# probcomp/PClean

Measured on AMD Instinct MI355X. Metric: rows/sec per Gibbs sweep on 1M-row synthetic hospital; F1 vs ground truth, higher is better.
Workload: dtype f64

## Files before the change

### pclean_amd/csrc/commit.hip

```cpp
#include <hip/hip_runtime.h>

#include <algorithm>
#include <cmath>

#define PCC_DEVICE
__device__ long long pcc_prof_t[64];
__device__ int pcc_prof_n;
#define PCC_STAMP(name)                                                   \
  do {                                                                    \
    if (tid == 0 && blockIdx.x == 0 && pcc_prof_n < 64) pcc_prof_t[pcc_prof_n++] = (long long)wall_clock64(); \
  } while (0)
#define PCC_CUR_SEPARATE
#include "commit_core.h"
#include "sweep_state.h"

struct PccRefresh {
  const int64_t* counts;
  double* logc_full;
  double* logc_m1;
  const double* lut;
  int32_t lut_n, stride;
};
struct PccRefreshAll {
  PccRefresh t[PCC_MAX_SLOTS];
};
struct PccSums {
  unsigned long long total[PCC_MAX_SLOTS], live[PCC_MAX_SLOTS], maxc[PCC_MAX_SLOTS];
  int32_t lut_overflow, pad;
};

struct CommitSlot {
  int table_id = -1;
  int stride = 0;
  bool state_set = false;
  DevBuf<uint8_t> live;
  DevBuf<int32_t> free_stack, gflag, gscan, glist, origin, chg;
  DevBuf<double> lut;
  int lut_n = 0;
  double lut_discount = 0.0;
  bool lut_valid = false;
  int64_t max_count = 0;
};

struct CommitState {
  bool enabled = false;
  int n_slots = 0, n_blocks = 0, n_plans = 0;
  int slot_of_table[PCLEAN_MAX_TABLES];
  int plan_block[PCC_MAX_BLOCKS];
  CommitSlot slot[PCC_MAX_SLOTS];
  PccTable h_tables[PCC_MAX_SLOTS];
  PccPlan h_plans[PCC_MAX_BLOCKS];
  DevBuf<PccTable> d_tables;
  DevBuf<PccPlan> d_plans;
  DevBuf<PccBlock> d_blocks;
  DevBuf<int32_t> d_colmap[PCC_MAX_BLOCKS];
  DevBuf<int32_t> d_states;
  bool tables_dirty = true, plans_dirty = true;
  int kcap[PCC_MAX_BLOCKS];
  DevBuf<int32_t> ht[PCC_MAX_BLOCKS], rep[PCC_MAX_BLOCKS], flags[PCC_MAX_BLOCKS], scan[PCC_MAX_BLOCKS], base[PCC_MAX_BLOCKS],
      newid[PCC_MAX_BLOCKS], recpos[PCC_MAX_BLOCKS];
  DevBuf<PccResult> d_res;
  DevBuf<PccSums> d_sums;
  DevBuf<int> d_bar;
  int bar_count = 0;
  int cap_m[PCC_MAX_BLOCKS] = {0}, cap_k[PCC_MAX_BLOCKS] = {0};
  DevBuf<int32_t> seg, seg_all, g_counts2;
  DevBuf<int32_t> g_moved[PCC_MAX_BLOCKS], g_choice[PCC_MAX_BLOCKS], g_new[PCC_MAX_BLOCKS], g_chosen[PCC_MAX_BLOCKS],
      g_vals[PCC_MAX_BLOCKS];
  DevBuf<PccBlock> d_blocks_g;
  PccBlock* h_blocks_g = nullptr;
  int32_t* h_g_counts2 = nullptr;
  PccBlock* h_blocks = nullptr;
  PccResult* h_res = nullptr;
  PccSums* h_sums = nullptr;
  int32_t* h_states = nullptr;
};

static CommitState* cst(pclean_ctx* ctx) {
  if (!ctx->commit_state) ctx->commit_state = new CommitState();
  return (CommitState*)ctx->commit_state;
}

void pclean_commit_state_free(pclean_ctx* ctx) {
  if (!ctx->commit_state) return;
  CommitState* c = (CommitState*)ctx->commit_state;
  for (auto& s : c->slot) {
    s.live.release(); s.free_stack.release(); s.gflag.release(); s.gscan.release(); s.glist.release(); s.origin.release(); s.chg.release();
    s.lut.release();
  }
  c->d_tables.release(); c->d_plans.release(); c->d_blocks.release(); c->d_states.release(); c->d_res.release();
  c->d_sums.release();
  c->d_bar.release();
  for (int b = 0; b < PCC_MAX_BLOCKS; ++b) {
    c->d_colmap[b].release(); c->ht[b].release(); c->rep[b].release(); c->flags[b].release(); c->scan[b].release();
    c->base[b].release(); c->newid[b].release(); c->recpos[b].release();
  }
  if (c->h_blocks) (void)hipHostFree(c->h_blocks);
  if (c->h_res) (void)hipHostFree(c->h_res);
  if (c->h_sums) (void)hipHostFree(c->h_sums);
  if (c->h_states) (void)hipHostFree(c->h_states);
  if (c->h_blocks_g) (void)hipHostFree(c->h_blocks_g);
  if (c->h_g_counts2) (void)hipHostFree(c->h_g_counts2);
  c->seg.release(); c->seg_all.release(); c->g_counts2.release(); c->d_blocks_g.release();
  for (int b = 0; b < PCC_MAX_BLOCKS; ++b) {
    c->g_moved[b].release(); c->g_choice[b].release(); c->g_new[b].release(); c->g_chosen[b].release(); c->g_vals[b].release();
  }
  ctx->dev_cur.release();
  delete c;
  ctx->commit_state = nullptr;
}

void pclean_commit_table_reuploaded(pclean_ctx* ctx, int table_id) {
  if (!ctx->commit_state || table_id < 0 || table_id >= PCLEAN_MAX_TABLES) return;
  CommitState* c = (CommitState*)ctx->commit_state;
  if (!c->enabled) return;
  const int si = c->slot_of_table[table_id];
  if (si >= 0) c->slot[si].state_set = false;
}

__global__ __launch_bounds__(1024) void pcc_commit_kernel(PccTable* tb, int n_slots, const PccPlan* plans, const PccBlock* blocks,
                                                          int n_blocks, PccResult* res, int gathered) {
  __shared__ int32_t part[1025];
  if (threadIdx.x == 0) pcc_prof_n = 0;
  if (threadIdx.x == 0 && !gathered) res->fallback_in = 0;
  if (threadIdx.x == 0)
    for (int s = 0; s < n_slots; ++s) {
      tb[s].state[PCC_ST_COLS_CHANGED] = 0;
      tb[s].state[PCC_ST_CREATED] = 0;
      tb[s].state[PCC_ST_DELETED] = 0;
      tb[s].state[PCC_ST_NCHG] = 0;
    }
  pcc_commit(tb, n_slots, plans, blocks, n_blocks, res, part, (int)threadIdx.x, (int)blockDim.x);
}

__device__ void pcc_mw_barrier(int* ctr, int target) {
  __syncthreads();
  if (threadIdx.x == 0) {
    __threadfence();
    atomicAdd(ctr, 1);
    while (__hip_atomic_load(ctr, __ATOMIC_RELAXED, __HIP_MEMORY_SCOPE_AGENT) < target) __builtin_amdgcn_s_sleep(1);
    __threadfence();
  }
  __syncthreads();
}
__global__ __launch_bounds__(1024) void pcc_commit_mw_kernel(PccTable* tb, int n_slots, const PccPlan* plans, const PccBlock* blocks,
                                                             int n_blocks, PccResult* res, int gathered, int* bar, int bar0) {
  __shared__ int32_t part[1025];
  const int tid = (int)threadIdx.x, nt = (int)blockDim.x, bi = (int)blockIdx.x;
  if (bi == 0 && tid == 0) {
    pcc_prof_n = 0;
    if (!gathered) res->fallback_in = 0;
    for (int s = 0; s < n_slots; ++s) {
      tb[s].state[PCC_ST_COLS_CHANGED] = 0;
      tb[s].state[PCC_ST_CREATED] = 0;
      tb[s].state[PCC_ST_DELETED] = 0;
      tb[s].state[PCC_ST_NCHG] = 0;
    }
    res->fallback = res->fallback_in;
    res->n_changed = 0;
    for (int s = 0; s < PCC_MAX_SLOTS; ++s) res->alloc_upper[s] = 0;
    for (int b = 0; b < PCC_MAX_BLOCKS; ++b) res->n_records[b] = res->n_distinct[b] = res->n_nested[b] = 0;
  }
  pcc_mw_barrier(bar, bar0 + n_blocks);
  if (res->fallback) {
    if (tid == 0) atomicAdd(bar, 1);
    return;
  }
  pcc_prepare_block(tb, plans[bi], blocks[bi], bi, res, tid, nt);
  __syncthreads();
  if (tid == 0) {
    const PccPlan& pl = plans[bi];
    for (int u = 0; u < pl.n_used; ++u) {
      const int s = pl.used_slot[u];
      const int a = res->alloc_upper[s];
      if (a == 0) continue;
      if (tb[s].state[PCC_ST_NHW] + (a > tb[s].state[PCC_ST_NFREE] ? a - tb[s].state[PCC_ST_NFREE] : 0) > tb[s].stride)
        atomicOr(&res->fallback, PCC_FB_CAPACITY);
    }
  }
  pcc_mw_barrier(bar, bar0 + 2 * n_blocks);
  if (res->fallback) return;
  pcc_apply_block(tb, plans[bi], blocks[bi], bi, res, part, tid, nt);
}

__global__ __launch_bounds__(256) void pcc_cur_kernel(const PccBlock* blocks, const PccResult* res) {
  if (res->fallback) return;
  pcc_update_cur(blocks[blockIdx.y], (int)(blockIdx.x * 256 + threadIdx.x), (int)(gridDim.x * 256));
}

struct PccGathered {
  int32_t* g_moved[PCC_MAX_BLOCKS];
  int32_t* g_choice[PCC_MAX_BLOCKS];
  int32_t* g_new[PCC_MAX_BLOCKS];
  int32_t* g_chosen[PCC_MAX_BLOCKS];
  int32_t* g_vals[PCC_MAX_BLOCKS];
  int32_t cap_out_m[PCC_MAX_BLOCKS], cap_out_k[PCC_MAX_BLOCKS];
};
__global__ __launch_bounds__(256) void pcc_pack_kernel(PccSegLayout L, const PccBlock* blocks, int empty, int32_t* seg) {
  pcc_pack(L, (int)blockIdx.y, blocks[blockIdx.y], empty, seg, (int)(blockIdx.x * 256 + threadIdx.x), (int)(gridDim.x * 256));
}
__global__ __launch_bounds__(256) void pcc_merge_kernel(PccSegLayout L, int n_ranks, const int32_t* all, PccGathered g,
                                                        int32_t* counts2, PccResult* res) {
  const int p = blockIdx.y;
  pcc_merge(L, p, n_ranks, all, g.cap_out_m[p], g.cap_out_k[p], g.g_moved[p], g.g_choice[p], g.g_new[p], g.g_chosen[p], g.g_vals[p],
            counts2 + 2 * p, &res->fallback_in, (int)(blockIdx.x * 256 + threadIdx.x), (int)(gridDim.x * 256),
            blockIdx.x == 0 ? counts2 + 2 * PCC_MAX_BLOCKS + 2 * p : nullptr);
}

__global__ void pcc_live_kernel(int n, const int64_t* counts, uint8_t* live) {
  const int r = blockIdx.x * blockDim.x + threadIdx.x;
  if (r < n) live[r] = counts[r] > 0 ? 1 : 0;
}

// ... 80 lines not shown
  for (int s = 0; s < sc->n_slots; ++s) {
    c->slot[s].table_id = sc->slot_table[s];
    c->h_tables[s] = sc->tables[s];
  }
  for (int p = 0; p < sc->n_plans; ++p) {
    c->plan_block[p] = sc->plan_block[p];
    c->h_plans[p] = sc->plans[p];
    const Block& b = ctx->block[sc->plan_block[p]];
    if (c->d_colmap[p].alloc(std::max<size_t>(b.colmap.size(), 2))) {
      delete sc;
      return pclean_fail(ctx, PCLEAN_ERR_HIP, "device alloc failed");
    }
    if (!b.colmap.empty()) {
      const hipError_t e = hipMemcpy(c->d_colmap[p].p, b.colmap.data(), b.colmap.size() * 4, hipMemcpyHostToDevice);
      if (e != hipSuccess) {
        delete sc;
        return pclean_fail(ctx, PCLEAN_ERR_HIP, "hipMemcpy failed: %s", hipGetErrorString(e));
      }
    }
    c->h_plans[p].colmap = c->d_colmap[p].p;
    c->kcap[p] = 0;
  }
  delete sc;
  if (c->d_tables.alloc(PCC_MAX_SLOTS) || c->d_plans.alloc(PCC_MAX_BLOCKS) || c->d_blocks.alloc(PCC_MAX_BLOCKS) ||
      c->d_states.alloc(PCC_MAX_SLOTS * PCC_ST_WORDS) || c->d_res.alloc(1) || c->d_sums.alloc(1))
    return pclean_fail(ctx, PCLEAN_ERR_HIP, "device alloc failed");
  if (!c->h_blocks) {
    HIPCHK(ctx, hipHostMalloc((void**)&c->h_blocks, sizeof(PccBlock) * PCC_MAX_BLOCKS, hipHostMallocDefault));
    HIPCHK(ctx, hipHostMalloc((void**)&c->h_res, sizeof(PccResult), hipHostMallocDefault));
    HIPCHK(ctx, hipHostMalloc((void**)&c->h_sums, sizeof(PccSums), hipHostMallocDefault));
    HIPCHK(ctx, hipHostMalloc((void**)&c->h_states, sizeof(int32_t) * PCC_MAX_SLOTS * PCC_ST_WORDS, hipHostMallocDefault));
  }
  c->tables_dirty = c->plans_dirty = true;
  c->enabled = true;
  *supported = 1;
  return PCLEAN_OK;
}

extern "C" int pclean_commit_n_slots(pclean_ctx* ctx, int32_t* n_slots, int32_t* table_ids) {
  if (!ctx || !n_slots) return PCLEAN_ERR_ARG;
  CommitState* c = cst(ctx);
  *n_slots = c->enabled ? c->n_slots : 0;
  if (table_ids)
    for (int s = 0; s < *n_slots; ++s) table_ids[s] = c->slot[s].table_id;
  return PCLEAN_OK;
}

extern "C" int pclean_commit_set_table_state(pclean_ctx* ctx, int32_t table_id, int32_t n_hw, int32_t n_free,
                                             const int32_t* free_stack) {
  if (!ctx || table_id < 0 || table_id >= PCLEAN_MAX_TABLES || n_hw < 0 || n_free < 0 || (n_free > 0 && !free_stack))
    return pclean_fail(ctx, PCLEAN_ERR_ARG, "pclean_commit_set_table_state: bad arguments");
  CommitState* c = cst(ctx);
  if (!c->enabled || c->slot_of_table[table_id] < 0)
    return pclean_fail(ctx, PCLEAN_ERR_STATE, "pclean_commit_set_table_state: table %d is not part of an enabled commit", table_id);
  HIPCHK(ctx, hipSetDevice(ctx->device));
  const int si = c->slot_of_table[table_id];
  CommitSlot& s = c->slot[si];
  CandTable& t = ctx->cand[table_id];
  if (!t.valid || n_hw > t.n_rows || n_free > n_hw)
    return pclean_fail(ctx, PCLEAN_ERR_ARG, "pclean_commit_set_table_state: table %d: %d rows in use, capacity %d", table_id, n_hw,
                       t.n_rows);
  const size_t st = std::max(t.n_rows, 1);
  if (s.live.alloc(st) || s.free_stack.alloc(st) || s.gflag.alloc(st) || s.gscan.alloc(st) || s.glist.alloc(st) ||
      s.origin.alloc(4 * st) || s.chg.alloc(st))
    return pclean_fail(ctx, PCLEAN_ERR_HIP, "device alloc failed");
  s.stride = t.n_rows;
// ... 68 lines not shown
  HIPCHK(ctx, hipMemcpyAsync(state8, c->d_states.p + (size_t)si * PCC_ST_WORDS, PCC_ST_WORDS * 4, hipMemcpyDeviceToHost, ctx->stream));
  if (cols && st) HIPCHK(ctx, hipMemcpyAsync(cols, t.cols.p, st * t.n_cols * 4, hipMemcpyDeviceToHost, ctx->stream));
  if (counts && st) HIPCHK(ctx, hipMemcpyAsync(counts, t.counts.p, st * 8, hipMemcpyDeviceToHost, ctx->stream));
  if (live && st) HIPCHK(ctx, hipMemcpyAsync(live, s.live.p, st, hipMemcpyDeviceToHost, ctx->stream));
  if (free_stack && st) HIPCHK(ctx, hipMemcpyAsync(free_stack, s.free_stack.p, st * 4, hipMemcpyDeviceToHost, ctx->stream));
  if (origin && st) {
    HIPCHK(ctx, hipMemcpyAsync(origin, s.origin.p, st * 16, hipMemcpyDeviceToHost, ctx->stream));
    HIPCHK(ctx, hipMemsetAsync(s.origin.p, 0, st * 16, ctx->stream));
  }
  HIPCHK(ctx, hipStreamSynchronize(ctx->stream));
  if (cols && st && t.h_cols_stale && t.h_cols.size() == st * (size_t)t.n_cols) {
    memcpy(t.h_cols.data(), cols, st * (size_t)t.n_cols * 4);
    t.h_cols_stale = false;
  }
  return PCLEAN_OK;
}

static int ensure_lut(pclean_ctx* ctx, CommitSlot& s, int64_t need) {
  const CandTable& t = ctx->cand[s.table_id];
  if (s.lut_valid && s.lut_discount == t.discount && s.lut_n > need) return PCLEAN_OK;
  const int64_t n = std::max<int64_t>(4096, 2 * need + 1024);
  if (n > (int64_t)1 << 30) return pclean_fail(ctx, PCLEAN_ERR_CAPACITY, "reference count beyond the log table");
  if (s.lut.alloc((size_t)n)) return pclean_fail(ctx, PCLEAN_ERR_HIP, "device alloc failed");
  std::vector<double> h((size_t)n);
  h[0] = -INFINITY;
  for (int64_t cc = 1; cc < n; ++cc) h[(size_t)cc] = std::log((double)cc - t.discount);
  HIPCHK(ctx, hipMemcpy(s.lut.p, h.data(), (size_t)n * sizeof(double), hipMemcpyHostToDevice));
  s.lut_n = (int)n;
  s.lut_discount = t.discount;
  s.lut_valid = true;
  return PCLEAN_OK;
}

static int launch_refresh(pclean_ctx* ctx, CommitState* c) {
  PccRefreshAll ra{};
  int max_stride = 1;
  for (int si = 0; si < c->n_slots; ++si) {
    CommitSlot& s = c->slot[si];
    CandTable& t = ctx->cand[s.table_id];
    ra.t[si] = PccRefresh{t.counts.p, t.logc_full.p, t.logc_m1.p, s.lut.p, s.lut_n, t.n_rows};
    max_stride = std::max(max_stride, t.n_rows);
  }
  { const int rcz = dev_zero(ctx, c->d_sums.p, sizeof(PccSums)); if (rcz) return rcz; }
  hipLaunchKernelGGL(pcc_refresh_kernel, dim3((max_stride + 255) / 256, c->n_slots), dim3(256), 0, ctx->stream, ra, c->d_res.p,
                     c->d_sums.p);
  {
    const int rcs = d2h_small(ctx, c->h_sums, c->d_sums.p, sizeof(PccSums));
    if (rcs) return rcs;
  }
  return PCLEAN_OK;
}

static int commit_device_impl(pclean_ctx* ctx, int32_t n_blocks, uint32_t sweep_idx, bool dist, bool local_empty,
                              int32_t max_local_rows, pclean_commit_summary* out);
extern "C" int pclean_commit_device(pclean_ctx* ctx, int32_t n_blocks, uint32_t sweep_idx, pclean_commit_summary* out) {
  if (ctx && ctx->comm_ranks > 1)
    return pclean_fail(ctx, PCLEAN_ERR_STATE, "pclean_commit_device: several ranks commit through pclean_commit_device_dist "
                                              "(every rank's moved rows and new-row records are gathered on the device first)");
  return commit_device_impl(ctx, n_blocks, sweep_idx, false, false, 0, out);
}
extern "C" int pclean_commit_device_dist(pclean_ctx* ctx, int32_t n_blocks, uint32_t sweep_idx, int32_t local_empty,
                                         int32_t max_local_rows, pclean_commit_summary* out) {
  if (!ctx || !ctx->rccl_comm || ctx->comm_ranks < 1 || max_local_rows < 0)
    return pclean_fail(ctx, PCLEAN_ERR_STATE, "pclean_commit_device_dist: pclean_comm_init first");
  return commit_device_impl(ctx, n_blocks, sweep_idx, true, local_empty != 0, max_local_rows, out);
}
static int commit_device_impl(pclean_ctx* ctx, int32_t n_blocks, uint32_t sweep_idx, bool dist, bool local_empty,
                              int32_t max_local_rows, pclean_commit_summary* out) {
  if (!ctx || !out) return pclean_fail(ctx, PCLEAN_ERR_ARG, "pclean_commit_device: bad arguments");
  CommitState* c = cst(ctx);
  SweepState* s = st(ctx);
  if (!c->enabled || c->n_blocks != n_blocks) return pclean_fail(ctx, PCLEAN_ERR_STATE, "pclean_commit_device: pclean_commit_enable first");
  if (!local_empty && (!s->outputs_pending || !s->last_dev_cur || s->last_blocks != n_blocks))
    return pclean_fail(ctx, PCLEAN_ERR_STATE, "pclean_commit_device: needs a pclean_sweep with device-resident referents "
                                              "(cur == NULL) and deferred outputs right before it");
  if (dist && (!ctx->dev_cur_valid || ctx->dev_cur_blocks != n_blocks))
// ... 14 lines not shown
        const int32_t* ov = ctx->cand[b.nodes[i].table].cols.p;
        if (pl.opt_vals[i] != ov) {
          pl.opt_vals[i] = ov;
          c->plans_dirty = true;
        }
      }
  }
  for (int si = 0; si < c->n_slots; ++si) {
    CandTable& t = ctx->cand[c->slot[si].table_id];
    PccTable& pt = c->h_tables[si];
    if (pt.cols != t.cols.p || pt.counts != t.counts.p) {
      pt.cols = t.cols.p;
      pt.counts = t.counts.p;
      c->tables_dirty = true;
    }
    int rc = ensure_lut(ctx, c->slot[si], c->slot[si].max_count + 1);
    if (rc) return rc;
  }
  if (c->tables_dirty) {
    HIPCHK(ctx, hipMemcpyAsync(c->d_tables.p, c->h_tables, sizeof(PccTable) * PCC_MAX_SLOTS, hipMemcpyHostToDevice, ctx->stream));
    HIPCHK(ctx, hipStreamSynchronize(ctx->stream));
    c->tables_dirty = false;
  }
  if (c->plans_dirty) {
    HIPCHK(ctx, hipMemcpyAsync(c->d_plans.p, c->h_plans, sizeof(PccPlan) * PCC_MAX_BLOCKS, hipMemcpyHostToDevice, ctx->stream));
    HIPCHK(ctx, hipStreamSynchronize(ctx->stream));
    c->plans_dirty = false;
  }
  for (int p = 0; p < c->n_plans; ++p) {
    const int bi = c->plan_block[p];
    const Block& b = ctx->block[bi];
    BlockRun& r = s->run[bi];
    const PccPlan& pl = c->h_plans[p];
    if (c->kcap[p] < 16384) c->kcap[p] = 16384;
    const int kcap = c->kcap[p];
    int hsz = 1;
    while (hsz < 4 * kcap) hsz <<= 1;
    if (c->ht[p].alloc(hsz) || c->rep[p].alloc(kcap) || c->flags[p].alloc(kcap) || c->scan[p].alloc(kcap) ||
        c->base[p].alloc((size_t)kcap * pl.n_used) || c->newid[p].alloc(kcap) || c->recpos[p].alloc(kcap))
      return pclean_fail(ctx, PCLEAN_ERR_HIP, "device alloc failed");
    PccBlock& pb = c->h_blocks[p];
    pb.N = N;
    pb.nn = (int)b.nodes.size();
    pb.block_id = bi;
    pb.sweep_idx = (int32_t)sweep_idx;
    pb.row_lo = (int32_t)(s->row_offset + ctx->active_begin);
    pb.pad0 = 0;
    pb.choice = r.choice.p;
    pb.chosen = s->chosen.p;
    pb.chosen_newpos = r.chosen_newpos.p;
    pb.vals = r.vals.p;
    pb.moved_list = r.moved_list.p;
    pb.new_list = r.new_list.p;
    pb.counts2 = s->tail_counts.p + 2 * bi;
    pb.cur = local_empty ? nullptr : const_cast<int32_t*>(s->last_cur_base) + (size_t)bi * s->last_cur_ld;
    pb.moved_choice = nullptr;
    pb.rec_chosen = nullptr;
    pb.delta = ctx->cand[b.nodes[0].table].stats.p;
    pb.kcap = kcap;
    pb.hmask = hsz - 1;
    pb.ht = c->ht[p].p;
    pb.rep = c->rep[p].p;
    pb.flags = c->flags[p].p;
    pb.scan = c->scan[p].p;
    pb.base = c->base[p].p;
    pb.newid = c->newid[p].p;
    pb.recpos = c->recpos[p].p;
  }
  HIPCHK(ctx, hipMemcpyAsync(c->d_blocks.p, c->h_blocks, sizeof(PccBlock) * c->n_plans, hipMemcpyHostToDevice, ctx->stream));
  const PccBlock* commit_blocks = c->d_blocks.p;
  bool stats_reduced = false;
  int cur_rows = N;
  if (dist) {
    PccSegLayout L{};
    L.n_plans = c->n_plans;
    int32_t off = 0;
    for (int p = 0; p < c->n_plans; ++p) {
      if (c->cap_m[p] <= 0) c->cap_m[p] = std::max(max_local_rows, 16);
      if (c->cap_k[p] <= 0) c->cap_k[p] = std::max(max_local_rows, 16);
      L.off[p] = off;
      L.cap_m[p] = c->cap_m[p];
      L.cap_k[p] = c->cap_k[p];
      L.nn[p] = (int)ctx->block[c->plan_block[p]].nodes.size();
      off += pcc_seg_words(L.cap_m[p], L.cap_k[p], L.nn[p]);
    }
    L.seg_words = off;
    if (c->seg.alloc((size_t)off) || c->seg_all.alloc((size_t)off * world) || c->g_counts2.alloc(4 * PCC_MAX_BLOCKS) ||
        c->d_blocks_g.alloc(PCC_MAX_BLOCKS))
      return pclean_fail(ctx, PCLEAN_ERR_HIP, "device alloc failed");
    if (!c->h_blocks_g) {
      HIPCHK(ctx, hipHostMalloc((void**)&c->h_blocks_g, sizeof(PccBlock) * PCC_MAX_BLOCKS, hipHostMallocDefault));
      HIPCHK(ctx, hipHostMalloc((void**)&c->h_g_counts2, sizeof(int32_t) * 4 * PCC_MAX_BLOCKS, hipHostMallocDefault));
    }
    PccGathered G{};
    for (int p = 0; p < c->n_plans; ++p) {
      const size_t om = (size_t)L.cap_m[p] * world, ok = (size_t)L.cap_k[p] * world;
      if (c->g_moved[p].alloc(om) || c->g_choice[p].alloc(om) || c->g_new[p].alloc(ok) || c->g_chosen[p].alloc(ok) ||
          c->g_vals[p].alloc(ok * L.nn[p]))
        return pclean_fail(ctx, PCLEAN_ERR_HIP, "device alloc failed");
      G.g_moved[p] = c->g_moved[p].p;
      G.g_choice[p] = c->g_choice[p].p;
      G.g_new[p] = c->g_new[p].p;
// ... 34 lines not shown
      pb.chosen_newpos = nullptr;
      pb.vals = c->g_vals[p].p;
      pb.moved_list = c->g_moved[p].p;
      pb.new_list = c->g_new[p].p;
      pb.moved_choice = c->g_choice[p].p;
      pb.rec_chosen = c->g_chosen[p].p;
      pb.counts2 = c->g_counts2.p + 2 * p;
      pb.cur = ctx->dev_cur.p + (size_t)bi * ctx->n_rows;
    }
    HIPCHK(ctx, hipMemcpyAsync(c->d_blocks_g.p, c->h_blocks_g, sizeof(PccBlock) * c->n_plans, hipMemcpyHostToDevice, ctx->stream));
    { const int rcz = dev_zero(ctx, c->d_res.p, sizeof(PccResult)); if (rcz) return rcz; }
    int32_t tids[PCC_MAX_BLOCKS];
    int n_t = 0;
    for (int p = 0; p < c->n_plans; ++p) {
      const int t = ctx->block[c->plan_block[p]].nodes[0].table;
      bool seen = false;
      for (int k = 0; k < n_t; ++k) seen |= tids[k] == t;
      if (!seen) tids[n_t++] = t;
    }
    int rc = pclean_comm_allreduce_stats_queue(ctx, n_t, tids, local_empty ? 1 : 0);
    if (rc) return rc;
    stats_reduced = true;
    hipLaunchKernelGGL(pcc_pack_kernel, dim3(64, c->n_plans), dim3(256), 0, ctx->stream, L, c->d_blocks.p, local_empty ? 1 : 0,
                       c->seg.p);
    rc = pclean_comm_allgather_i32(ctx, c->seg.p, c->seg_all.p, (size_t)L.seg_words);
    if (rc) return rc;
    hipLaunchKernelGGL(pcc_merge_kernel, dim3(64, c->n_plans), dim3(256), 0, ctx->stream, L, world, c->seg_all.p, G, c->g_counts2.p,
                       c->d_res.p);
    HIPCHK(ctx, hipMemcpyAsync(c->h_g_counts2, c->g_counts2.p, sizeof(int32_t) * 4 * PCC_MAX_BLOCKS, hipMemcpyDeviceToHost, ctx->stream));
    commit_blocks = c->d_blocks_g.p;
    cur_rows = 0;
    for (int p = 0; p < c->n_plans; ++p) cur_rows = std::max<int64_t>(cur_rows, (int64_t)L.cap_m[p] * world);
  }
  static const bool no_mw = getenv("PCLEAN_COMMIT_ONE_WG") != nullptr;
  bool all_exclusive = c->n_plans > 1 && !no_mw;
  for (int p = 0; p < c->n_plans; ++p) all_exclusive = all_exclusive && c->h_plans[p].exclusive != 0;
  if (all_exclusive && !c->d_bar.p) {
    if (c->d_bar.alloc(16)) return pclean_fail(ctx, PCLEAN_ERR_HIP, "device alloc failed");
    HIPCHK(ctx, hipMemsetAsync(c->d_bar.p, 0, 16 * sizeof(int), ctx->stream));
    c->bar_count = 0;
  }
  if (all_exclusive) {
    if (c->bar_count > (1 << 30)) {
      HIPCHK(ctx, hipMemsetAsync(c->d_bar.p, 0, 16 * sizeof(int), ctx->stream));
      c->bar_count = 0;
    }
    hipLaunchKernelGGL(pcc_commit_mw_kernel, dim3(c->n_plans), dim3(1024), 0, ctx->stream, c->d_tables.p, c->n_slots, c->d_plans.p,
                       commit_blocks, c->n_plans, c->d_res.p, dist ? 1 : 0, c->d_bar.p, c->bar_count);
    c->bar_count += 2 * c->n_plans;
  } else {
    hipLaunchKernelGGL(pcc_commit_kernel, dim3(1), dim3(1024), 0, ctx->stream, c->d_tables.p, c->n_slots, c->d_plans.p,
                       commit_blocks, c->n_plans, c->d_res.p, dist ? 1 : 0);
  }
  hipLaunchKernelGGL(pcc_cur_kernel, dim3(std::max(1, std::min(1024, (cur_rows + 255) / 256)), c->n_plans), dim3(256), 0, ctx->stream,
                     commit_blocks, c->d_res.p);
  int rc = launch_refresh(ctx, c);
  if (rc) return rc;
  rc = d2h_small(ctx, c->h_res, c->d_res.p, sizeof(PccResult));
  if (!rc) rc = d2h_small(ctx, c->h_states, c->d_states.p, sizeof(int32_t) * PCC_MAX_SLOTS * PCC_ST_WORDS);
  if (rc) return rc;
  rc = pclean_sweep_finish_queue(ctx);
  if (!rc) rc = d2h_flush(ctx);
  if (rc) return rc;
  HIPCHK(ctx, hipGetLastError());
  HIPCHK(ctx, hipStreamSynchronize(ctx->stream));
  rc = pclean_sweep_finish_synced(ctx);
  if (rc) return rc;
  static const bool prof = getenv("PCLEAN_COMMIT_PROF") != nullptr;
  if (prof) {
    long long t[64];
    int n = 0;
    (void)hipMemcpyFromSymbol(&n, HIP_SYMBOL(pcc_prof_n), sizeof n);
    (void)hipMemcpyFromSymbol(t, HIP_SYMBOL(pcc_prof_t), sizeof t);
    fprintf(stderr, "[pclean] commit kernel phases (us since start; 100 MHz clock):");
    for (int i = 1; i < n && i < 64; ++i) fprintf(stderr, " %.1f", (double)(t[i] - t[0]) / 100.0);
    fprintf(stderr, "  (records %d %d, moved %d %d)\n", c->h_res->n_records[0], c->h_res->n_records[1], s->h_counts[0], s->h_counts[2]);
  }
  out->fallback = c->h_res->fallback;
  out->n_changed = c->h_res->n_changed;
  out->n_slots = c->n_slots;
  out->stats_reduced = stats_reduced ? 1 : 0;
  for (int p = 0; p < c->n_plans; ++p) {
    out->n_records[c->plan_block[p]] = c->h_res->n_records[p];
    out->n_distinct[c->plan_block[p]] = c->h_res->n_distinct[p];
    if (2 * c->h_res->n_records[p] > c->kcap[p]) c->kcap[p] = 2 * c->h_res->n_records[p];
    if (dist) {
      c->cap_m[p] = out->fallback ? 0 : std::max(1024, 4 * c->h_g_counts2[2 * PCC_MAX_BLOCKS + 2 * p] + 256);
      c->cap_k[p] = out->fallback ? 0 : std::max(256, 4 * c->h_g_counts2[2 * PCC_MAX_BLOCKS + 2 * p + 1] + 256);
    }
  }
  if (dist && !out->fallback) {
    int64_t moved = 0;
    for (int p = 0; p < c->n_plans; ++p) moved += c->h_g_counts2[2 * p];
    out->n_changed = (int32_t)moved;
  }
  if (out->fallback) return PCLEAN_OK;
  for (int guard = 0; c->h_sums->lut_overflow && guard < 4; ++guard) {
    for (int si = 0; si < c->n_slots; ++si) {
      rc = ensure_lut(ctx, c->slot[si], (int64_t)c->h_sums->maxc[si] + 1);
      if (rc) return rc;
    }
// ... 47 lines not shown
```

### pclean_amd/csrc/commit_core.h

```cpp
#pragma once
#include <stdint.h>

#ifdef PCC_DEVICE
#define PCC_FN __device__
#define PCC_BARRIER() __syncthreads()
#define PCC_ADD64(p, v) atomicAdd((unsigned long long*)(p), (unsigned long long)(long long)(v))
#define PCC_ADD32(p, v) atomicAdd((int*)(p), (int)(v))
#define PCC_FETCH_ADD32(p, v) atomicAdd((int*)(p), (int)(v))
#define PCC_OR32(p, v) atomicOr((int*)(p), (int)(v))
#define PCC_MIN32(p, v) atomicMin((int*)(p), (int)(v))
#define PCC_CAS32(p, cmp, v) atomicCAS((int*)(p), (int)(cmp), (int)(v))
#else
#define PCC_FN static inline
#define PCC_BARRIER() ((void)0)
#define PCC_ADD64(p, v) (*(p) += (int64_t)(v))
#define PCC_ADD32(p, v) (*(p) += (int32_t)(v))
static inline int32_t pcc_fetch_add32_host(int32_t* p, int32_t v) {
  const int32_t old = *p;
  *p += v;
  return old;
}
#define PCC_FETCH_ADD32(p, v) pcc_fetch_add32_host((p), (v))
#define PCC_OR32(p, v) (*(p) |= (int32_t)(v))
#define PCC_MIN32(p, v) (*(p) = (*(p) < (int32_t)(v) ? *(p) : (int32_t)(v)))
// ... 270 lines not shown
      fr_slot[depth] = t.fk_slot[q];
      fr_n[depth] = L2;
      fr_next[depth] = 0;
      ++depth;
    }
  }
}

PCC_FN void pcc_mark_reuse(const PccTable* tb, const PccPlan& pl, const PccBlock& b, int k, bool pending_delta, int tid, int nt) {
  const PccTable& root = tb[pl.used_slot[0]];
  for (int j = tid; j < k; j += nt) {
    int32_t fl = b.flags[j];
    int32_t fresh = 0;
    if ((fl & PCC_F_FIRST) && (fl & PCC_F_SIMPLE)) {
      const int32_t* v = pcc_record(b, j);
      int32_t row[PCC_MAX_NODES];
      (void)pcc_new_nodes(pl, v, row);
      const int old = b.cur[b.new_list[j]];
      bool same = old >= 0 && root.live[old] && root.counts[old] + (pending_delta ? b.delta[old] : 0) == 0;
      for (int c = 0; c < root.n_cols && same; ++c)
        same = root.cols[(size_t)c * root.stride + old] == pcc_col_value(tb, pl, v, row, 0, c);
      if (same) {
        b.newid[j] = old;
        b.flags[j] = fl | PCC_F_REUSE;
      } else {
        fresh = 1;
      }
    }
    b.scan[j] = fresh;
  }
  PCC_BARRIER();
}

PCC_FN void pcc_prepare_block(const PccTable* tb, const PccPlan& pl, const PccBlock& b, int bi, PccResult* res, int tid, int nt) {
  const int k = b.counts2[1];
  if (tid == 0) {
    res->n_records[bi] = k;
    res->n_distinct[bi] = 0;
    res->n_nested[bi] = 0;
  }
  if (k > b.kcap) {
    if (tid == 0) PCC_OR32(&res->fallback, PCC_FB_RECORDS);
    return;
  }
  if (k == 0) return;
  for (int j = tid; j < k; j += nt) b.recpos[j] = b.chosen_newpos ? b.chosen_newpos[b.new_list[j]] : j;
  int hm = b.hmask < 63 ? b.hmask : 63;
  while (hm + 1 < 4 * k && hm < b.hmask) hm = 2 * hm + 1;
  const uint32_t hmask = (uint32_t)hm;
  for (int i = tid; i <= hm; i += nt) b.ht[i] = -1;
  PCC_BARRIER();
  for (int j = tid; j < k; j += nt) {
    const int32_t* v = pcc_record(b, j);
    uint32_t s = pcc_hash(b, v) & hmask;
    for (;;) {
      int32_t c = b.ht[s];
      if (c < 0) {
        c = PCC_CAS32(&b.ht[s], -1, j);
        if (c < 0) break;
      }
      if (pcc_same(b, pcc_record(b, c), v)) {
        PCC_MIN32(&b.ht[s], j);
        break;
      }
      s = (s + 1) & hmask;
    }
  }
  PCC_BARRIER();
  for (int j = tid; j < k; j += nt) {
    const int32_t* v = pcc_record(b, j);
    uint32_t s = pcc_hash(b, v) & hmask;
    for (;;) {
      const int32_t c = b.ht[s];
      if (pcc_same(b, pcc_record(b, c), v)) {
        b.rep[j] = c;
        break;
      }
      s = (s + 1) & hmask;
    }
    int32_t fl = 0;
    if (b.rep[j] == j) {
      fl = PCC_F_FIRST | PCC_F_SIMPLE;
      int32_t row[PCC_MAX_NODES];
      const uint64_t mask = pcc_new_nodes(pl, v, row);
      if (mask != 1ull) {
        fl &= ~PCC_F_SIMPLE;
        PCC_ADD32(&res->n_nested[bi], 1);
      }
      for (int p = 0; p < pl.n_fk_nodes; ++p) {
        const int f = pl.fk_post[p];
        if (((mask >> f) & 1ull) && !(f == 0 && pl.exclusive)) PCC_ADD32(&res->alloc_upper[pl.slot[f]], 1);
      }
      for (int l = 0; l < pl.n_nodes; ++l)
        if (pl.kind[l] == 1 && pl.dummy_val[l] != 0 && ((mask >> pl.parent[l]) & 1ull) && v[l] >= 0 &&
            pl.opt_vals[l][v[l]] == pl.dummy_val[l] - 1)
          PCC_OR32(&res->fallback, PCC_FB_DUMMY);
      PCC_ADD32(&res->n_distinct[bi], 1);
    }
    b.flags[j] = fl;
  }
  PCC_BARRIER();
  if (pl.exclusive) {
    pcc_mark_reuse(tb, pl, b, k, true, tid, nt);
    for (int j = tid; j < k; j += nt)
      if ((b.flags[j] & PCC_F_FIRST) && !(b.flags[j] & PCC_F_REUSE)) PCC_ADD32(&res->alloc_upper[pl.used_slot[0]], 1);
    PCC_BARRIER();
  }
}

PCC_FN void pcc_update_cur(const PccBlock& b, int tid, int nt) {
  const int k = b.counts2[1], n_moved = b.counts2[0];
  for (int m = tid; m < n_moved; m += nt) {
    const int r = b.moved_list[m];
    const int c = b.moved_choice ? b.moved_choice[m] : b.choice[r];
    if (c >= 0) b.cur[r] = c;
  }
  for (int j = tid; j < k; j += nt) b.cur[b.new_list[j]] = b.newid[j];
}

PCC_FN void pcc_apply_block(PccTable* tb, const PccPlan& pl, const PccBlock& b, int bi, PccResult* res, int32_t* part, int tid,
                            int nt) {
  const int k = b.counts2[1], n_moved = b.counts2[0];
  const int U = pl.n_used;
  PccTable& root = tb[pl.used_slot[0]];
  {
    const int n0 = root.state[PCC_ST_NHW];
    for (int r = tid; r < n0; r += nt) root.counts[r] += b.delta[r];
    PCC_BARRIER();
  }
  PCC_STAMP("delta");
  if (k > 0) {
  if (!pl.exclusive) pcc_mark_reuse(tb, pl, b, k, false, tid, nt);
  const int32_t n_simple = pcc_excl_scan(b.scan, k, part, tid, nt);
  for (int j = tid; j < k; j += nt) b.base[(size_t)j * U] = b.scan[j];
  PCC_BARRIER();
  PCC_STAMP("reuse+scan");
  int32_t total[PCC_MAX_SLOTS];
  for (int u = 0; u < U; ++u) total[u] = u == 0 ? n_simple : 0;
  if (res->n_nested[bi] > 0)
  for (int u = 0; u < U; ++u) {
// ... 150 lines not shown
      for (int r = 0; r < n_ranks; ++r) {
        const int32_t* o = all + (size_t)r * L.seg_words + L.off[p];
        mm = o[0] > mm ? o[0] : mm;
        mk = o[1] > mk ? o[1] : mk;
      }
      rank_max[0] = mm;
      rank_max[1] = mk;
    }
  }
  if (bad) return;
  int base_m = 0, base_k = 0;
  for (int r = 0; r < n_ranks; ++r) {
    const int32_t* o = all + (size_t)r * L.seg_words + L.off[p];
    const int32_t* mrow = o + 4;
    const int32_t* mch = mrow + cm;
    const int32_t* nrow = mch + cm;
    const int32_t* nchs = nrow + ck;
    const int32_t* rec = nchs + ck;
    const int nm = o[0], nk = o[1];
    for (int m = tid; m < nm; m += nt) {
      g_moved[base_m + m] = mrow[m];
      g_choice[base_m + m] = mch[m];
    }
    for (int j = tid; j < nk; j += nt) {
      g_new[base_k + j] = nrow[j];
      g_chosen[base_k + j] = nchs[j];
    }
    for (int x = tid; x < nk * nn; x += nt) g_vals[(size_t)base_k * nn + x] = rec[x];
    base_m += nm;
    base_k += nk;
  }
}

PCC_FN void pcc_commit(PccTable* tb, int n_slots, const PccPlan* plans, const PccBlock* blocks, int n_blocks, PccResult* res,
                       int32_t* part, int tid, int nt) {
  if (tid == 0) {
    res->fallback = res->fallback_in;
    res->n_changed = 0;
    for (int s = 0; s < PCC_MAX_SLOTS; ++s) res->alloc_upper[s] = 0;
    for (int bi = 0; bi < PCC_MAX_BLOCKS; ++bi) res->n_records[bi] = res->n_distinct[bi] = res->n_nested[bi] = 0;
  }
  PCC_BARRIER();
  PCC_STAMP("start");
  if (res->fallback) return;
  for (int bi = 0; bi < n_blocks; ++bi) {
    pcc_prepare_block(tb, plans[bi], blocks[bi], bi, res, tid, nt);
    PCC_STAMP("prepare");
  }
  PCC_BARRIER();
  if (tid == 0)
    for (int s = 0; s < n_slots; ++s) {
      const int a = res->alloc_upper[s];
      if (a == 0) continue;
      const int from_free = tb[s].n_blocks_using <= 1 ? tb[s].state[PCC_ST_NFREE] : 0;
      if (tb[s].state[PCC_ST_NHW] + (a > from_free ? a - from_free : 0) > tb[s].stride) res->fallback |= PCC_FB_CAPACITY;
    }
  PCC_BARRIER();
  if (res->fallback) return;
  for (int bi = 0; bi < n_blocks; ++bi) pcc_apply_block(tb, plans[bi], blocks[bi], bi, res, part, tid, nt);
}

#ifndef PCC_DEVICE_ONLY
struct PccNodeIn {
  int32_t kind, table, child_begin, n_children, parent, parent_fk_col, colmap_begin, dummy_value;
};
static inline void pcc_post_order(const PccNodeIn* nodes, const int32_t* children, int f, PccPlan& pl) {
  for (int c = 0; c < nodes[f].n_children; ++c) {
    const int g = children[nodes[f].child_begin + c];
    if (nodes[g].kind == 0) pcc_post_order(nodes, children, g, pl);
  }
  pl.fk_post[pl.n_fk_nodes++] = f;
}
static inline int pcc_build_plan(const PccNodeIn* nodes, int n_nodes, const int32_t* children, const int32_t* slot_of_table,
                                 PccPlan& pl) {
  if (n_nodes > PCC_MAX_NODES || n_nodes < 1 || nodes[0].kind != 0) return -1;
  pl.n_nodes = n_nodes;
  pl.n_fk_nodes = 0;
  pl.n_used = 0;
  pl.track = 0;
  for (int i = 0; i < n_nodes; ++i) {
    pl.kind[i] = nodes[i].kind;
    pl.parent[i] = nodes[i].parent;
    pl.parent_fk_col[i] = nodes[i].parent_fk_col;
    pl.cmb[i] = nodes[i].colmap_begin;
    pl.dummy_val[i] = nodes[i].kind == 1 ? nodes[i].dummy_value : 0;
    pl.slot[i] = -1;
    pl.node_used[i] = -1;
    pl.opt_vals[i] = nullptr;
    if (nodes[i].kind == 1 && nodes[i].dummy_value != 0) pl.track = 1;
    if (nodes[i].kind == 0) {
      const int s = slot_of_table[nodes[i].table];
      if (s < 0) return -2;
// ... 137 lines not shown
```

Before: 408.2 million.

## Split commit prepare phase into grid-wide kernels and skip redundant block uploads

The per-block prepare step (hash-table init, insert, classify, reuse marking) used to run inside the single-workgroup or one-WG-per-block commit kernel. It now runs as three grid-wide kernels launched across many workgroups, and the commit kernel only does the apply phase. The prep-init kernel also zeroes the sums buffer, replacing a separate memset, and the host skips re-uploading the PccBlock descriptors when they are unchanged. The cost is two extra kernel launches and a host-side memcmp. The old narrow path is kept behind an environment variable.

```diff
diff --git a/pclean_amd/csrc/commit.hip b/pclean_amd/csrc/commit.hip
--- a/pclean_amd/csrc/commit.hip
+++ b/pclean_amd/csrc/commit.hip
@@ -6,9 +6,10 @@
 #define PCC_DEVICE
 __device__ long long pcc_prof_t[64];
 __device__ int pcc_prof_n;
+__device__ int pcc_prof_wg;
 #define PCC_STAMP(name)                                                   \
   do {                                                                    \
-    if (tid == 0 && blockIdx.x == 0 && pcc_prof_n < 64) pcc_prof_t[pcc_prof_n++] = (long long)wall_clock64(); \
+    if (tid == 0 && (int)blockIdx.x == pcc_prof_wg && pcc_prof_n < 64) pcc_prof_t[pcc_prof_n++] = (long long)wall_clock64(); \
   } while (0)
 #define PCC_CUR_SEPARATE
 #include "commit_core.h"
@@ -63,6 +64,8 @@
   DevBuf<PccSums> d_sums;
   DevBuf<int> d_bar;
   int bar_count = 0;
+  PccBlock up_blocks[PCC_MAX_BLOCKS];
+  int up_n = -1;
   int cap_m[PCC_MAX_BLOCKS] = {0}, cap_k[PCC_MAX_BLOCKS] = {0};
   DevBuf<int32_t> seg, seg_all, g_counts2;
   DevBuf<int32_t> g_moved[PCC_MAX_BLOCKS], g_choice[PCC_MAX_BLOCKS], g_new[PCC_MAX_BLOCKS], g_chosen[PCC_MAX_BLOCKS],
@@ -118,19 +121,59 @@
   if (si >= 0) c->slot[si].state_set = false;
 }
 
+__device__ void pcc_start(PccTable* tb, int n_slots, PccResult* res, int gathered) {
+  pcc_prof_n = 0;
+  if (!gathered) res->fallback_in = 0;
+  for (int s = 0; s < n_slots; ++s) {
+    tb[s].state[PCC_ST_COLS_CHANGED] = 0;
+    tb[s].state[PCC_ST_CREATED] = 0;
+    tb[s].state[PCC_ST_DELETED] = 0;
+    tb[s].state[PCC_ST_NCHG] = 0;
+  }
+}
+
+#define PCC_PREP_WG 256
+__global__ __launch_bounds__(PCC_PREP_WG) void pcc_prep_init_kernel(PccTable* tb, int n_slots, PccBlock* blocks, int n_blocks,
+                                                                    PccResult* res, int gathered, int sweep_idx, unsigned* sums,
+                                                                    int sums_words) {
+  const int tid = (int)(blockIdx.x * PCC_PREP_WG + threadIdx.x), nt = (int)(gridDim.x * PCC_PREP_WG), bi = (int)blockIdx.y;
+  const int refused = gathered ? res->fallback_in : 0;
+  if (bi == 0 && tid == 0) {
+    pcc_start(tb, n_slots, res, gathered);
+    pcc_reset_result(res);
+    for (int p = 0; p < n_blocks; ++p) {
+      blocks[p].sweep_idx = sweep_idx;
+      if (!refused) pcc_prepare_counts(blocks[p], p, res);
+    }
+  }
+  if (bi == 0)
+    for (int i = tid; i < sums_words; i += nt) sums[i] = 0u;
+  if (refused) return;
+  pcc_prepare_init(blocks[bi], tid, nt);
+}
+__global__ __launch_bounds__(PCC_PREP_WG) void pcc_prep_insert_kernel(const PccBlock* blocks, const PccResult* res) {
+  if (res->fallback_in) return;
+  pcc_prepare_insert(blocks[blockIdx.y], (int)(blockIdx.x * PCC_PREP_WG + threadIdx.x), (int)(gridDim.x * PCC_PREP_WG));
+}
+__global__ __launch_bounds__(PCC_PREP_WG) void pcc_prep_classify_kernel(const PccTable* tb, const PccPlan* plans, const PccBlock* blocks,
+                                                                        PccResult* res) {
+  if (res->fallback_in) return;
+  const int tid = (int)(blockIdx.x * PCC_PREP_WG + threadIdx.x), nt = (int)(gridDim.x * PCC_PREP_WG), bi = (int)blockIdx.y;
+  pcc_prepare_classify(plans[bi], blocks[bi], bi, res, tid, nt);
+  pcc_prepare_reuse(tb, plans[bi], blocks[bi], res, tid, nt);
+}
+
 __global__ __launch_bounds__(1024) void pcc_commit_kernel(PccTable* tb, int n_slots, const PccPlan* plans, const PccBlock* blocks,
-                                                          int n_blocks, PccResult* res, int gathered) {
+                                                          int n_blocks, PccResult* res, int gathered, int prepared) {
   __shared__ int32_t part[1025];
-  if (threadIdx.x == 0) pcc_prof_n = 0;
-  if (threadIdx.x == 0 && !gathered) res->fallback_in = 0;
-  if (threadIdx.x == 0)
-    for (int s = 0; s < n_slots; ++s) {
-      tb[s].state[PCC_ST_COLS_CHANGED] = 0;
-      tb[s].state[PCC_ST_CREATED] = 0;
-      tb[s].state[PCC_ST_DELETED] = 0;
-      tb[s].state[PCC_ST_NCHG] = 0;
-    }
-  pcc_commit(tb, n_slots, plans, blocks, n_blocks, res, part, (int)threadIdx.x, (int)blockDim.x);
+  const int tid = (int)threadIdx.x, nt = (int)blockDim.x;
+  if (prepared) {
+    PCC_STAMP("start");
+    pcc_commit_apply(tb, n_slots, plans, blocks, n_blocks, res, part, tid, nt);
+    return;
+  }
+  if (tid == 0) pcc_start(tb, n_slots, res, gathered);
+  pcc_commit(tb, n_slots, plans, blocks, n_blocks, res, part, tid, nt);
 }
 
 __device__ void pcc_mw_barrier(int* ctr, int target) {
@@ -144,30 +187,25 @@
   __syncthreads();
 }
 __global__ __launch_bounds__(1024) void pcc_commit_mw_kernel(PccTable* tb, int n_slots, const PccPlan* plans, const PccBlock* blocks,
-                                                             int n_blocks, PccResult* res, int gathered, int* bar, int bar0) {
+                                                             int n_blocks, PccResult* res, int gathered, int* bar, int bar0,
+                                                             int prepared) {
   __shared__ int32_t part[1025];
   const int tid = (int)threadIdx.x, nt = (int)blockDim.x, bi = (int)blockIdx.x;
-  if (bi == 0 && tid == 0) {
-    pcc_prof_n = 0;
-    if (!gathered) res->fallback_in = 0;
-    for (int s = 0; s < n_slots; ++s) {
-      tb[s].state[PCC_ST_COLS_CHANGED] = 0;
-      tb[s].state[PCC_ST_CREATED] = 0;
-      tb[s].state[PCC_ST_DELETED] = 0;
-      tb[s].state[PCC_ST_NCHG] = 0;
-    }
-    res->fallback = res->fallback_in;
-    res->n_changed = 0;
-    for (int s = 0; s < PCC_MAX_SLOTS; ++s) res->alloc_upper[s] = 0;
-    for (int b = 0; b < PCC_MAX_BLOCKS; ++b) res->n_records[b] = res->n_distinct[b] = res->n_nested[b] = 0;
-  }
-  pcc_mw_barrier(bar, bar0 + n_blocks);
-  if (res->fallback) {
-    if (tid == 0) atomicAdd(bar, 1);
-    return;
-  }
-  pcc_prepare_block(tb, plans[bi], blocks[bi], bi, res, tid, nt);
-  __syncthreads();
+  if (prepared) {
+    PCC_STAMP("start");
+  } else {
+    if (bi == 0 && tid == 0) {
+      pcc_start(tb, n_slots, res, gathered);
+      pcc_reset_result(res);
+    }
+    pcc_mw_barrier(bar, bar0 + n_blocks);
+    if (res->fallback_in) {
+      if (tid == 0) atomicAdd(bar, 1);
+      return;
+    }
+    pcc_prepare_block(tb, plans[bi], blocks[bi], bi, res, tid, nt);
+    __syncthreads();
+  }
   if (tid == 0) {
     const PccPlan& pl = plans[bi];
     for (int u = 0; u < pl.n_used; ++u) {
@@ -178,7 +216,7 @@
         atomicOr(&res->fallback, PCC_FB_CAPACITY);
     }
   }
-  pcc_mw_barrier(bar, bar0 + 2 * n_blocks);
+  pcc_mw_barrier(bar, bar0 + (prepared ? 1 : 2) * n_blocks);
   if (res->fallback) return;
   pcc_apply_block(tb, plans[bi], blocks[bi], bi, res, part, tid, nt);
 }
@@ -325,6 +363,7 @@
     HIPCHK(ctx, hipHostMalloc((void**)&c->h_states, sizeof(int32_t) * PCC_MAX_SLOTS * PCC_ST_WORDS, hipHostMallocDefault));
   }
   c->tables_dirty = c->plans_dirty = true;
+  c->up_n = -1;
   c->enabled = true;
   *supported = 1;
   return PCLEAN_OK;
@@ -459,7 +498,7 @@
   return PCLEAN_OK;
 }
 
-static int launch_refresh(pclean_ctx* ctx, CommitState* c) {
+static int launch_refresh(pclean_ctx* ctx, CommitState* c, bool zeroed = false) {
   PccRefreshAll ra{};
   int max_stride = 1;
   for (int si = 0; si < c->n_slots; ++si) {
@@ -468,7 +507,7 @@
     ra.t[si] = PccRefresh{t.counts.p, t.logc_full.p, t.logc_m1.p, s.lut.p, s.lut_n, t.n_rows};
     max_stride = std::max(max_stride, t.n_rows);
   }
-  { const int rcz = dev_zero(ctx, c->d_sums.p, sizeof(PccSums)); if (rcz) return rcz; }
+  if (!zeroed) { const int rcz = dev_zero(ctx, c->d_sums.p, sizeof(PccSums)); if (rcz) return rcz; }
   hipLaunchKernelGGL(pcc_refresh_kernel, dim3((max_stride + 255) / 256, c->n_slots), dim3(256), 0, ctx->stream, ra, c->d_res.p,
                      c->d_sums.p);
   {
@@ -549,7 +588,8 @@
     const Block& b = ctx->block[bi];
     BlockRun& r = s->run[bi];
     const PccPlan& pl = c->h_plans[p];
-    if (c->kcap[p] < 16384) c->kcap[p] = 16384;
+    static const int kcap_min = getenv("PCLEAN_COMMIT_KCAP") ? std::max(1, atoi(getenv("PCLEAN_COMMIT_KCAP"))) : 16384;
+    if (c->kcap[p] < kcap_min) c->kcap[p] = kcap_min;
     const int kcap = c->kcap[p];
     int hsz = 1;
     while (hsz < 4 * kcap) hsz <<= 1;
@@ -584,7 +624,20 @@
     pb.newid = c->newid[p].p;
     pb.recpos = c->recpos[p].p;
   }
-  HIPCHK(ctx, hipMemcpyAsync(c->d_blocks.p, c->h_blocks, sizeof(PccBlock) * c->n_plans, hipMemcpyHostToDevice, ctx->stream));
+  static const bool no_mw = getenv("PCLEAN_COMMIT_ONE_WG") != nullptr;
+  static const bool narrow = no_mw || getenv("PCLEAN_COMMIT_NARROW") != nullptr;
+  {
+    bool same = !narrow && c->up_n == c->n_plans;
+    for (int p = 0; p < c->n_plans; ++p) {
+      PccBlock x = c->h_blocks[p];
+      x.sweep_idx = 0;
+      same = same && memcmp(&x, &c->up_blocks[p], sizeof x) == 0;
+      c->up_blocks[p] = x;
+    }
+    c->up_n = c->n_plans;
+    if (!same)
+      HIPCHK(ctx, hipMemcpyAsync(c->d_blocks.p, c->h_blocks, sizeof(PccBlock) * c->n_plans, hipMemcpyHostToDevice, ctx->stream));
+  }
   const PccBlock* commit_blocks = c->d_blocks.p;
   bool stats_reduced = false;
   int cur_rows = N;
@@ -685,9 +738,32 @@
     cur_rows = 0;
     for (int p = 0; p < c->n_plans; ++p) cur_rows = std::max<int64_t>(cur_rows, (int64_t)L.cap_m[p] * world);
   }
-  static const bool no_mw = getenv("PCLEAN_COMMIT_ONE_WG") != nullptr;
   bool all_exclusive = c->n_plans > 1 && !no_mw;
   for (int p = 0; p < c->n_plans; ++p) all_exclusive = all_exclusive && c->h_plans[p].exclusive != 0;
+  static const bool prof = getenv("PCLEAN_COMMIT_PROF") != nullptr;
+  if (prof) {
+    const char* w = getenv("PCLEAN_COMMIT_PROF_WG");
+    const int wg = all_exclusive && w ? std::max(0, std::min(atoi(w), c->n_plans - 1)) : 0;
+    (void)hipMemcpyToSymbol(HIP_SYMBOL(pcc_prof_wg), &wg, sizeof wg);
+  }
+  if (!narrow) {
+    int kmax = 1, hmax = 1;
+    for (int p = 0; p < c->n_plans; ++p) {
+      kmax = std::max(kmax, c->kcap[p]);
+      int hsz = 1;
+      while (hsz < 4 * c->kcap[p]) hsz <<= 1;
+      hmax = std::max(hmax, hsz);
+    }
+    const dim3 g_rec((unsigned)((kmax + PCC_PREP_WG - 1) / PCC_PREP_WG), (unsigned)c->n_plans);
+    const dim3 g_init((unsigned)((std::max(kmax, hmax) + PCC_PREP_WG - 1) / PCC_PREP_WG), (unsigned)c->n_plans);
+    static_assert(sizeof(PccSums) % sizeof(unsigned) == 0, "pcc_prep_init_kernel clears the sums word by word");
+    hipLaunchKernelGGL(pcc_prep_init_kernel, g_init, dim3(PCC_PREP_WG), 0, ctx->stream, c->d_tables.p, c->n_slots,
+                       const_cast<PccBlock*>(commit_blocks), c->n_plans, c->d_res.p, dist ? 1 : 0, (int)sweep_idx,
+                       (unsigned*)c->d_sums.p, (int)(sizeof(PccSums) / sizeof(unsigned)));
+    hipLaunchKernelGGL(pcc_prep_insert_kernel, g_rec, dim3(PCC_PREP_WG), 0, ctx->stream, commit_blocks, c->d_res.p);
+    hipLaunchKernelGGL(pcc_prep_classify_kernel, g_rec, dim3(PCC_PREP_WG), 0, ctx->stream, c->d_tables.p, c->d_plans.p, commit_blocks,
+                       c->d_res.p);
+  }
   if (all_exclusive && !c->d_bar.p) {
     if (c->d_bar.alloc(16)) return pclean_fail(ctx, PCLEAN_ERR_HIP, "device alloc failed");
     HIPCHK(ctx, hipMemsetAsync(c->d_bar.p, 0, 16 * sizeof(int), ctx->stream));
@@ -699,15 +775,15 @@
       c->bar_count = 0;
     }
     hipLaunchKernelGGL(pcc_commit_mw_kernel, dim3(c->n_plans), dim3(1024), 0, ctx->stream, c->d_tables.p, c->n_slots, c->d_plans.p,
-                       commit_blocks, c->n_plans, c->d_res.p, dist ? 1 : 0, c->d_bar.p, c->bar_count);
-    c->bar_count += 2 * c->n_plans;
+                       commit_blocks, c->n_plans, c->d_res.p, dist ? 1 : 0, c->d_bar.p, c->bar_count, narrow ? 0 : 1);
+    c->bar_count += (narrow ? 2 : 1) * c->n_plans;
   } else {
     hipLaunchKernelGGL(pcc_commit_kernel, dim3(1), dim3(1024), 0, ctx->stream, c->d_tables.p, c->n_slots, c->d_plans.p,
-                       commit_blocks, c->n_plans, c->d_res.p, dist ? 1 : 0);
+                       commit_blocks, c->n_plans, c->d_res.p, dist ? 1 : 0, narrow ? 0 : 1);
   }
   hipLaunchKernelGGL(pcc_cur_kernel, dim3(std::max(1, std::min(1024, (cur_rows + 255) / 256)), c->n_plans), dim3(256), 0, ctx->stream,
                      commit_blocks, c->d_res.p);
-  int rc = launch_refresh(ctx, c);
+  int rc = launch_refresh(ctx, c, !narrow);
   if (rc) return rc;
   rc = d2h_small(ctx, c->h_res, c->d_res.p, sizeof(PccResult));
   if (!rc) rc = d2h_small(ctx, c->h_states, c->d_states.p, sizeof(int32_t) * PCC_MAX_SLOTS * PCC_ST_WORDS);
@@ -719,7 +795,6 @@
   HIPCHK(ctx, hipStreamSynchronize(ctx->stream));
   rc = pclean_sweep_finish_synced(ctx);
   if (rc) return rc;
-  static const bool prof = getenv("PCLEAN_COMMIT_PROF") != nullptr;
   if (prof) {
     long long t[64];
     int n = 0;
diff --git a/pclean_amd/csrc/commit_core.h b/pclean_amd/csrc/commit_core.h
--- a/pclean_amd/csrc/commit_core.h
+++ b/pclean_amd/csrc/commit_core.h
@@ -326,24 +326,33 @@
   PCC_BARRIER();
 }
 
-PCC_FN void pcc_prepare_block(const PccTable* tb, const PccPlan& pl, const PccBlock& b, int bi, PccResult* res, int tid, int nt) {
-  const int k = b.counts2[1];
-  if (tid == 0) {
-    res->n_records[bi] = k;
-    res->n_distinct[bi] = 0;
-    res->n_nested[bi] = 0;
-  }
-  if (k > b.kcap) {
-    if (tid == 0) PCC_OR32(&res->fallback, PCC_FB_RECORDS);
-    return;
-  }
-  if (k == 0) return;
-  for (int j = tid; j < k; j += nt) b.recpos[j] = b.chosen_newpos ? b.chosen_newpos[b.new_list[j]] : j;
+
+PCC_FN int32_t pcc_hash_mask(const PccBlock& b, int k) {
   int hm = b.hmask < 63 ? b.hmask : 63;
   while (hm + 1 < 4 * k && hm < b.hmask) hm = 2 * hm + 1;
-  const uint32_t hmask = (uint32_t)hm;
+  return hm;
+}
+PCC_FN bool pcc_has_records(const PccBlock& b, int k) { return k > 0 && k <= b.kcap; }
+
+PCC_FN void pcc_prepare_counts(const PccBlock& b, int bi, PccResult* res) {
+  const int k = b.counts2[1];
+  res->n_records[bi] = k;
+  res->n_distinct[bi] = 0;
+  res->n_nested[bi] = 0;
+  if (k > b.kcap) PCC_OR32(&res->fallback, PCC_FB_RECORDS);
+}
+PCC_FN void pcc_prepare_init(const PccBlock& b, int tid, int nt) {
+  const int k = b.counts2[1];
+  if (!pcc_has_records(b, k)) return;
+  for (int j = tid; j < k; j += nt) b.recpos[j] = b.chosen_newpos ? b.chosen_newpos[b.new_list[j]] : j;
+  const int hm = pcc_hash_mask(b, k);
   for (int i = tid; i <= hm; i += nt) b.ht[i] = -1;
-  PCC_BARRIER();
+}
+
+PCC_FN void pcc_prepare_insert(const PccBlock& b, int tid, int nt) {
+  const int k = b.counts2[1];
+  if (!pcc_has_records(b, k)) return;
+  const uint32_t hmask = (uint32_t)pcc_hash_mask(b, k);
   for (int j = tid; j < k; j += nt) {
     const int32_t* v = pcc_record(b, j);
     uint32_t s = pcc_hash(b, v) & hmask;
@@ -360,7 +369,12 @@
       s = (s + 1) & hmask;
     }
   }
-  PCC_BARRIER();
+}
+
+PCC_FN void pcc_prepare_classify(const PccPlan& pl, const PccBlock& b, int bi, PccResult* res, int tid, int nt) {
+  const int k = b.counts2[1];
+  if (!pcc_has_records(b, k)) return;
+  const uint32_t hmask = (uint32_t)pcc_hash_mask(b, k);
   for (int j = tid; j < k; j += nt) {
     const int32_t* v = pcc_record(b, j);
     uint32_t s = pcc_hash(b, v) & hmask;
@@ -393,13 +407,26 @@
     }
     b.flags[j] = fl;
   }
-  PCC_BARRIER();
-  if (pl.exclusive) {
-    pcc_mark_reuse(tb, pl, b, k, true, tid, nt);
-    for (int j = tid; j < k; j += nt)
-      if ((b.flags[j] & PCC_F_FIRST) && !(b.flags[j] & PCC_F_REUSE)) PCC_ADD32(&res->alloc_upper[pl.used_slot[0]], 1);
-    PCC_BARRIER();
-  }
+}
+
+PCC_FN void pcc_prepare_reuse(const PccTable* tb, const PccPlan& pl, const PccBlock& b, PccResult* res, int tid, int nt) {
+  const int k = b.counts2[1];
+  if (!pl.exclusive || !pcc_has_records(b, k)) return;
+  pcc_mark_reuse(tb, pl, b, k, true, tid, nt);
+  for (int j = tid; j < k; j += nt)
+    if ((b.flags[j] & PCC_F_FIRST) && !(b.flags[j] & PCC_F_REUSE)) PCC_ADD32(&res->alloc_upper[pl.used_slot[0]], 1);
+}
+
+PCC_FN void pcc_prepare_block(const PccTable* tb, const PccPlan& pl, const PccBlock& b, int bi, PccResult* res, int tid, int nt) {
+  if (tid == 0) pcc_prepare_counts(b, bi, res);
+  pcc_prepare_init(b, tid, nt);
+  PCC_BARRIER();
+  pcc_prepare_insert(b, tid, nt);
+  PCC_BARRIER();
+  pcc_prepare_classify(pl, b, bi, res, tid, nt);
+  PCC_BARRIER();
+  pcc_prepare_reuse(tb, pl, b, res, tid, nt);
+  PCC_BARRIER();
 }
 
 PCC_FN void pcc_update_cur(const PccBlock& b, int tid, int nt) {
@@ -616,22 +643,14 @@
   }
 }
 
-PCC_FN void pcc_commit(PccTable* tb, int n_slots, const PccPlan* plans, const PccBlock* blocks, int n_blocks, PccResult* res,
-                       int32_t* part, int tid, int nt) {
-  if (tid == 0) {
-    res->fallback = res->fallback_in;
-    res->n_changed = 0;
-    for (int s = 0; s < PCC_MAX_SLOTS; ++s) res->alloc_upper[s] = 0;
-    for (int bi = 0; bi < PCC_MAX_BLOCKS; ++bi) res->n_records[bi] = res->n_distinct[bi] = res->n_nested[bi] = 0;
-  }
-  PCC_BARRIER();
-  PCC_STAMP("start");
-  if (res->fallback) return;
-  for (int bi = 0; bi < n_blocks; ++bi) {
-    pcc_prepare_block(tb, plans[bi], blocks[bi], bi, res, tid, nt);
-    PCC_STAMP("prepare");
-  }
-  PCC_BARRIER();
+PCC_FN void pcc_reset_result(PccResult* res) {
+  res->fallback = res->fallback_in;
+  res->n_changed = 0;
+  for (int s = 0; s < PCC_MAX_SLOTS; ++s) res->alloc_upper[s] = 0;
+  for (int bi = 0; bi < PCC_MAX_BLOCKS; ++bi) res->n_records[bi] = res->n_distinct[bi] = res->n_nested[bi] = 0;
+}
+PCC_FN void pcc_commit_apply(PccTable* tb, int n_slots, const PccPlan* plans, const PccBlock* blocks, int n_blocks, PccResult* res,
+                             int32_t* part, int tid, int nt) {
   if (tid == 0)
     for (int s = 0; s < n_slots; ++s) {
       const int a = res->alloc_upper[s];
@@ -642,6 +661,19 @@
   PCC_BARRIER();
   if (res->fallback) return;
   for (int bi = 0; bi < n_blocks; ++bi) pcc_apply_block(tb, plans[bi], blocks[bi], bi, res, part, tid, nt);
+}
+PCC_FN void pcc_commit(PccTable* tb, int n_slots, const PccPlan* plans, const PccBlock* blocks, int n_blocks, PccResult* res,
+                       int32_t* part, int tid, int nt) {
+  if (tid == 0) pcc_reset_result(res);
+  PCC_BARRIER();
+  PCC_STAMP("start");
+  if (res->fallback) return;
+  for (int bi = 0; bi < n_blocks; ++bi) {
+    pcc_prepare_block(tb, plans[bi], blocks[bi], bi, res, tid, nt);
+    PCC_STAMP("prepare");
+  }
+  PCC_BARRIER();
+  pcc_commit_apply(tb, n_slots, plans, blocks, n_blocks, res, part, tid, nt);
 }
 
 #ifndef PCC_DEVICE_ONLY
```

New measurement: 419.0 million (median of 6 runs). 1.03x the previous value.
